# davdwan21/Silent-Speech

Hardware: AMD Instinct MI355X
Metric: clips/sec (30-frame, fwd+bwd) (higher is better)
Workload: dtype f32; 1 GPU; BASELINE config 2: landmark (K=40, D=84) + 64x64 uint8 ROI CNN + 2-layer BiGRU(192), T=30, C=5, train step = fwd + CE(ls .05) + bwd + grad all-reduce + clip(1.0) + Adam, dropout on; batch_per_gpu=256, global_batch=256, frames=30, parallelism=dp1, micro_batches_in_flight=1

## Files before the change

### silent_speech_amd/csrc/gemm.hip

```cpp
#include <stdlib.h>

#define SS_STAMP_ROW ((int)(blockIdx.x + gridDim.x * (blockIdx.y + gridDim.y * blockIdx.z)))
#include "ss_common.h"

STAMP_TABLE(ss_debug_stamps_gemm)

namespace {

constexpr int BM = 128, BN = 64, BK = 16;
constexpr int LDK = BK + 4;
constexpr int LDM_A = BM + 4;
constexpr int LDM_B = BN + 4;

struct RowMap {
  int G, S, off;
  __device__ __forceinline__ long operator()(int r) const {
    if (G == 0x7fffffff) return r + off;
    return (long)(r / G) * S + (r % G) + off;
  }
};

struct GemmParams {
  const float* A;
  const float* B;
  float* C;
  const float* bias;
  int M, N, K;
  int lda, ldb, ldc;
  RowMap ra, rb;
  float* asum;
  int ksplit;
  int nz;
  long sA, sB, sC, sBias, sAsum;
  int kcat;
  int flags;
};

struct TileId { int bx, by, bz, gx, gy; };

__device__ __forceinline__ void gemm_epilogue(const GemmParams& p, f32x4 (&acc)[4][2], int m0, int n0, int zs, int wm, int wn,
                                              int i, int g, float* stage ,
                                              const TileId& id) {
  if (p.flags & 8) {
    f32x4* w = reinterpret_cast<f32x4*>(p.C) + (((long)id.bz * id.gy + id.by) * id.gx + id.bx) * (8 * 256) + threadIdx.x;
#pragma unroll
    for (int mt = 0; mt < 4; ++mt)
#pragma unroll
      for (int nt = 0; nt < 2; ++nt) w[(mt * 2 + nt) * 256] = acc[mt][nt];
    return;
  }
  const bool accumulate = p.flags & 1, relu = p.flags & 2;
  const bool atomic = p.nz > 1 || (p.flags & 4);
  auto emit = [&](const f32x4& av, int mt, int nt) {
    int col = n0 + wn * 32 + nt * 16 + i;
    if (col >= p.N) return;
    float bv = (p.bias && zs == 0) ? p.bias[col] : 0.f;
#pragma unroll
    for (int r = 0; r < 4; ++r) {
      int row = m0 + wm * 64 + mt * 16 + 4 * g + r;
      if (row >= p.M) continue;
      float v = av[r] + bv;
      float* dst = p.C + (long)row * p.ldc + col;
      if (atomic) {
        atomicAdd(dst, v);
      } else {
        if (accumulate) v += *dst;
        if (relu) v = relu_f(v);
        *dst = v;
      }
    }
  };
  if (stage && !atomic && n0 + BN <= p.N && (p.ldc & 3) == 0 && (reinterpret_cast<uintptr_t>(p.C) & 15) == 0) {
    constexpr int LDS_C = BN + 4;
    __syncthreads();
#pragma unroll
    for (int mt = 0; mt < 4; ++mt)
#pragma unroll
      for (int nt = 0; nt < 2; ++nt) {
        const int col = wn * 32 + nt * 16 + i;
        const float bv = (p.bias && zs == 0) ? p.bias[n0 + col] : 0.f;
#pragma unroll
        for (int r = 0; r < 4; ++r) stage[(wm * 64 + mt * 16 + 4 * g + r) * LDS_C + col] = acc[mt][nt][r] + bv;
      }
    __syncthreads();
    const int c4 = (threadIdx.x & 15) * 4, r0 = threadIdx.x >> 4;
#pragma unroll
    for (int it = 0; it < BM / 16; ++it) {
      const int row = r0 + 16 * it;
      if (m0 + row < p.M) {
        f32x4 v = *reinterpret_cast<const f32x4*>(&stage[row * LDS_C + c4]);
        f32x4* dst = reinterpret_cast<f32x4*>(p.C + (long)(m0 + row) * p.ldc + n0 + c4);
        if (accumulate) v += *dst;
        if (relu) {
#pragma unroll
          for (int e = 0; e < 4; ++e) v[e] = relu_f(v[e]);
        }
        *dst = v;
      }
    }
    return;
  }
// ... 380 lines not shown
    }
  }
  if (rem) {
    __syncthreads();
    da.tail(dlds, rem);
    db.tail(dlds + D_A, rem);
    __syncthreads();
    compute(dlds, -1);
  }
  }
  static_assert(BM * (BN + 4) <= DSTAGES * D_STAGE, "the output tile is staged in the k-tile ring");
  gemm_epilogue(p, acc, m0, n0, zs, wm, wn, i, g, dlds, id);
}

template <bool A_KC, bool B_KC>
__global__ __launch_bounds__(256, 3) void gemm_dma_kernel(GemmParams p) {
  extern __shared__ __attribute__((aligned(16))) float dlds[];
  gemm_dma_body<A_KC, B_KC>(p, TileId{(int)blockIdx.x, (int)blockIdx.y, (int)blockIdx.z, (int)gridDim.x, (int)gridDim.y}, dlds);
}

constexpr int GEMM_GROUP_MAX = 4;
struct GemmGroup {
  GemmParams p[GEMM_GROUP_MAX];
  int first[GEMM_GROUP_MAX + 1];
  int gx[GEMM_GROUP_MAX], gy[GEMM_GROUP_MAX];
  int n;
};

template <bool A_KC, bool B_KC>
__global__ __launch_bounds__(256, 3) void gemm_dma_group_kernel(GemmGroup gg) {
  extern __shared__ __attribute__((aligned(16))) float dlds[];
  int j = 0;
#pragma unroll
  for (int q = 1; q < GEMM_GROUP_MAX; ++q)
    if (q < gg.n && (int)blockIdx.x >= gg.first[q]) j = q;
  const int local = blockIdx.x - gg.first[j], gx = gg.gx[j], gy = gg.gy[j];
  const int bx = local % gx, by = (local / gx) % gy, bz = local / (gx * gy);
  gemm_dma_body<A_KC, B_KC>(gg.p[j], TileId{bx, by, bz, gx, gy}, dlds);
}

struct ReduceItem { const f32x4* ws; int nz, gx, gy, M, N; float* C; int ldc; long sC; };
struct ReduceGroup {
  ReduceItem it[GEMM_GROUP_MAX];
  int first[GEMM_GROUP_MAX + 1];
  int n;
};
__device__ __forceinline__ void splitk_reduce_body(const ReduceItem& r, int block) {
  const int q = block & 7, tile = block >> 3;
  const int bx = tile % r.gx, by = (tile / r.gx) % r.gy, bi = tile / (r.gx * r.gy);
  const int tid = threadIdx.x, lane = tid & 63, wid = tid >> 6, wm = wid >> 1, wn = wid & 1, i = lane & 15, g = lane >> 4;
  const int mt = q >> 1, nt = q & 1;
  const f32x4* src = r.ws + ((((long)bi * r.nz) * r.gy + by) * r.gx + bx) * (8 * 256) + q * 256 + tid;
  const long zstride = (long)r.gy * r.gx * (8 * 256);
  f32x4 s0 = {0.f, 0.f, 0.f, 0.f};
  int z = 0;
  for (; z + 8 <= r.nz; z += 8) {
    f32x4 v[8];
#pragma unroll
    for (int u = 0; u < 8; ++u) v[u] = src[(z + u) * zstride];
    s0 += ((v[0] + v[1]) + (v[2] + v[3])) + ((v[4] + v[5]) + (v[6] + v[7]));
  }
  {
    f32x4 v[8];
#pragma unroll
    for (int u = 0; u < 8; ++u) v[u] = (z + u < r.nz) ? src[(z + u) * zstride] : f32x4{0.f, 0.f, 0.f, 0.f};
    s0 += ((v[0] + v[1]) + (v[2] + v[3])) + ((v[4] + v[5]) + (v[6] + v[7]));
  }
  const int col = bx * BN + wn * 32 + nt * 16 + i;
  if (col >= r.N) return;
#pragma unroll
  for (int rr = 0; rr < 4; ++rr) {
    const int row = by * BM + wm * 64 + mt * 16 + 4 * g + rr;
    if (row < r.M) r.C[bi * r.sC + (long)row * r.ldc + col] += s0[rr];
  }
}
__global__ __launch_bounds__(256) void splitk_reduce_kernel(ReduceItem r) { splitk_reduce_body(r, blockIdx.x); }
__global__ __launch_bounds__(256) void splitk_reduce_group_kernel(ReduceGroup rg) {
  int j = 0;
#pragma unroll
  for (int q = 1; q < GEMM_GROUP_MAX; ++q)
    if (q < rg.n && (int)blockIdx.x >= rg.first[q]) j = q;
  splitk_reduce_body(rg.it[j], blockIdx.x - rg.first[j]);
}

namespace wide {
constexpr int WT = 192, WNT = 512, WNWV = 8;
constexpr int W_U = WT / 4;
constexpr int W_PIECES = WT * BK / 4 / 64;
constexpr int W_STAGE = 2 * WT * BK;
constexpr int W_LPW = 2 * W_PIECES / WNWV;
constexpr int W_Q = 18;
constexpr int W_SLAB = WT * WT;
static_assert(2 * W_PIECES % WNWV == 0, "pieces deal evenly over the waves");

struct WideProblem {
  const float *A, *B;
  float* C;
  int M, N, K, lda, ldb, ldc;
  RowMap ra, rb;
  int ksplit, nz, gx, gy, batch;
  long sA, sB, sC;
  long ws_off;
};
struct WideGroup {
  WideProblem p[GEMM_GROUP_MAX];
  int first[GEMM_GROUP_MAX + 1];
  int rfirst[GEMM_GROUP_MAX + 1];
  float* ws;
  int n;
};

#define WIDE_K_LOOP                                                                                                      \
  {                                                                                                                      \
    _Pragma("unroll") for (int s_ = 0; s_ < DSTAGES - 1; ++s_) if (s_ < nfull) issue(s_);                                \
    for (int t0 = 0; t0 < nfull; t0 += DSTAGES) {                                                                        \
      _Pragma("unroll") for (int s_ = 0; s_ < DSTAGES; ++s_) {                                                           \
        const int t = t0 + s_;                                                                                           \
        if (t < nfull) {                                                                                                 \
          if (t + DSTAGES - 2 < nfull) ss_vmcnt_wait<(DSTAGES - 2) * W_LPW>(); else ss_vmcnt_wait<0>();                  \
          ss_raw_barrier();                                                                                              \
          if (t + DSTAGES - 1 < nfull) issue((s_ + DSTAGES - 1) % DSTAGES);                                              \
          read(dlds + s_ * W_STAGE);                                                                                     \
          mma();                                                                                                         \
        }                                                                                                                \
      }                                                                                                                  \
    }                                                                                                                    \
  }

struct WidePieces {
  const float* src[W_LPW];
  int q[W_LPW], r[W_LPW];
  int G[W_LPW], S[W_LPW], ld[W_LPW];
  bool lin[W_LPW];
  __device__ __forceinline__ void init(const WideProblem& P, const float* A, const float* B, int m0, int n0, int kbeg) {
    const int lane = threadIdx.x & 63, wave = threadIdx.x >> 6;
#pragma unroll
    for (int n = 0; n < W_LPW; ++n) {
      const int piece = wave + WNWV * n;
      const bool isb = piece >= W_PIECES;
      const int sl = (piece - (isb ? W_PIECES : 0)) * 64 + lane;
      const int k = sl / W_U, u = sl % W_U;
      int ru = u - 4 * ((k >> 2) & 1);
      ru += ru < 0 ? W_U : 0;
      const RowMap& rm = isb ? P.rb : P.ra;
      const int nrows = isb ? P.N : P.M, row0 = isb ? n0 : m0;
      ld[n] = isb ? P.ldb : P.lda;
      lin[n] = rm.G == 0x7fffffff;
      G[n] = rm.G; S[n] = rm.S;
      const int gk = kbeg + k;
      src[n] = (isb ? B : A) + min(row0 + 4 * ru, nrows - 4) + (long)rm.off * ld[n];
      q[n] = lin[n] ? 0 : gk / rm.G;
      r[n] = gk - q[n] * rm.G;
      if (lin[n]) src[n] += (long)gk * ld[n];
    }
  }
  __device__ __forceinline__ const float* cur(int n) const { return lin[n] ? src[n] : src[n] + ((long)q[n] * S[n] + r[n]) * ld[n]; }
  __device__ __forceinline__ void issue(unsigned stage_byte) const {
    const int wave = threadIdx.x >> 6;
#pragma unroll
    for (int n = 0; n < W_LPW; ++n) ss_dma16(cur(n), stage_byte + (wave + WNWV * n) * 1024);
  }
  __device__ __forceinline__ void advance() {
#pragma unroll
// ... 38 lines not shown
  dp.init(P, P.A + bi * P.sA, P.B + bi * P.sB, m0, n0, kbeg);
  int offA[3], offB[6];
#pragma unroll
  for (int mt = 0; mt < 3; ++mt) {
    const int m = wm * 48 + mt * 16 + i;
    offA[mt] = 4 * g * WT + 4 * (((m >> 2) + 4 * (g & 1)) % W_U) + (m & 3);
  }
#pragma unroll
  for (int nt = 0; nt < 6; ++nt) {
    const int nn = wn * 96 + nt * 16 + i;
    offB[nt] = WT * BK + 4 * g * WT + 4 * (((nn >> 2) + 4 * (g & 1)) % W_U) + (nn & 3);
  }
  f32x4 acc[3][6];
#pragma unroll
  for (int mt = 0; mt < 3; ++mt)
#pragma unroll
    for (int nt = 0; nt < 6; ++nt) acc[mt][nt] = f32x4{0.f, 0.f, 0.f, 0.f};

  auto issue = [&](int buf) {
    dp.issue((unsigned)(buf * W_STAGE * 4));
    dp.advance();
  };
  float a[3][4], b[6][4];
  auto read = [&](const float* st) {
#pragma unroll
    for (int kk = 0; kk < 4; ++kk) {
#pragma unroll
      for (int mt = 0; mt < 3; ++mt) a[mt][kk] = st[offA[mt] + kk * WT];
#pragma unroll
      for (int nt = 0; nt < 6; ++nt) b[nt][kk] = st[offB[nt] + kk * WT];
    }
  };
  auto mma = [&]() {
#pragma unroll
    for (int kk = 0; kk < 4; ++kk)
#pragma unroll
      for (int mt = 0; mt < 3; ++mt)
#pragma unroll
        for (int nt = 0; nt < 6; ++nt) acc[mt][nt] = mfma16(a[mt][kk], b[nt][kk], acc[mt][nt]);
  };
  WIDE_K_LOOP
  if (rem) {
    __syncthreads();
    dp.tail(dlds, rem);
    __syncthreads();
    read(dlds);
    mma();
  }
  f32x4* w = reinterpret_cast<f32x4*>(gg.ws + P.ws_off) + (long)local * (W_Q * WNT) + threadIdx.x;
#pragma unroll
  for (int mt = 0; mt < 3; ++mt)
#pragma unroll
    for (int nt = 0; nt < 6; ++nt) w[(mt * 6 + nt) * WNT] = acc[mt][nt];
}

__global__ __launch_bounds__(WNT) void gemm_wide_reduce_kernel(WideGroup gg) {
  int j = 0;
#pragma unroll
  for (int q = 1; q < GEMM_GROUP_MAX; ++q)
    if (q < gg.n && (int)blockIdx.x >= gg.rfirst[q]) j = q;
  const WideProblem& P = gg.p[j];
  const int blk = blockIdx.x - gg.rfirst[j];
  const int q = blk % W_Q, tile = blk / W_Q;
  const int bx = tile % P.gx, by = (tile / P.gx) % P.gy, bi = tile / (P.gx * P.gy);
  const int tid = threadIdx.x, lane = tid & 63, wid = tid >> 6, wm = wid >> 1, wn = wid & 1, i = lane & 15, g = lane >> 4;
  const int mt = q / 6, nt = q % 6;
  const long tiles = (long)P.gx * P.gy;
  const f32x4* src = reinterpret_cast<const f32x4*>(gg.ws + P.ws_off) + (((long)bi * P.nz * tiles + by * P.gx + bx) * W_Q + q) * WNT + tid;
  const long zstride = tiles * W_Q * WNT;
  f32x4 s0 = {0.f, 0.f, 0.f, 0.f};
  int z = 0;
  for (; z + 8 <= P.nz; z += 8) {
    f32x4 v[8];
#pragma unroll
    for (int u = 0; u < 8; ++u) v[u] = src[(z + u) * zstride];
    s0 += ((v[0] + v[1]) + (v[2] + v[3])) + ((v[4] + v[5]) + (v[6] + v[7]));
  }
  {
    f32x4 v[8];
#pragma unroll
    for (int u = 0; u < 8; ++u) v[u] = (z + u < P.nz) ? src[(z + u) * zstride] : f32x4{0.f, 0.f, 0.f, 0.f};
    s0 += ((v[0] + v[1]) + (v[2] + v[3])) + ((v[4] + v[5]) + (v[6] + v[7]));
  }
  const int col = bx * WT + wn * 96 + nt * 16 + i;
  if (col >= P.N) return;
#pragma unroll
  for (int rr = 0; rr < 4; ++rr) {
    const int row = by * WT + wm * 48 + mt * 16 + 4 * g + rr;
    if (row < P.M) P.C[bi * P.sC + (long)row * P.ldc + col] += s0[rr];
  }
}

struct WideKcParams {
  const float *A, *B, *bias;
  float* C;
  int M, N, K, lda, ldb, ldc, gx, gy;
  long sA, sB, sC, sBias;
};
struct WidePiecesKc {
  const float* src[W_LPW];
  __device__ __forceinline__ void init(const WideKcParams& P, const float* A, const float* B, int m0, int n0) {
    const int lane = threadIdx.x & 63, wave = threadIdx.x >> 6;
#pragma unroll
    for (int n = 0; n < W_LPW; ++n) {
      const int piece = wave + WNWV * n;
      const bool isb = piece >= W_PIECES;
      const int sl = (piece - (isb ? W_PIECES : 0)) * 64 + lane;
      const int rr = sl >> 2, ku = (sl & 3) ^ kc_swz(rr);
      const int nrows = isb ? P.N : P.M, row0 = isb ? n0 : m0;
      const int gr = min(row0 + rr, nrows - 1);
      src[n] = (isb ? B + (long)gr * P.ldb : A + (long)gr * P.lda) + 4 * ku;
    }
  }
  __device__ __forceinline__ void issue(unsigned stage_byte) const {
    const int wave = threadIdx.x >> 6;
#pragma unroll
    for (int n = 0; n < W_LPW; ++n) ss_dma16(src[n], stage_byte + (wave + WNWV * n) * 1024);
  }
  __device__ __forceinline__ void advance() {
#pragma unroll
    for (int n = 0; n < W_LPW; ++n) src[n] += BK;
  }
  __device__ __forceinline__ void tail(float* img, int kvalid) const {
    const int lane = threadIdx.x & 63, wave = threadIdx.x >> 6;
#pragma unroll
    for (int n = 0; n < W_LPW; ++n) {
      const int piece = wave + WNWV * n;
      const int sl = (piece % W_PIECES) * 64 + lane;
      const int ku = (sl & 3) ^ kc_swz(sl >> 2);
      f32x4 v = {0.f, 0.f, 0.f, 0.f};
#pragma unroll
      for (int e = 0; e < 4; ++e)
        if (4 * ku + e < kvalid) v[e] = src[n][e];
      *reinterpret_cast<f32x4*>(img + piece * 256 + 4 * lane) = v;
    }
  }
// ... 79 lines not shown
    }
  }
}
}

int splitk_slices(int K, int splits, int* per_out) {
  const int per = ceil_div(ceil_div(K, splits), BK * KSUB) * BK * KSUB;
  if (per_out) *per_out = per;
  return ceil_div(K, per);
}

}

extern "C" int ss_gemm_splitk_ws_floats(int M, int N, int K, int splits, int batch, long* floats) {
  SS_REQUIRE(M > 0 && N > 0 && K > 0 && splits >= 1 && batch >= 1 && floats, SS_ERR_ARG);
  *floats = (long)batch * splitk_slices(K, splits, nullptr) * ceil_div(M, BM) * ceil_div(N, BN) * BM * BN;
  return SS_OK;
}

extern "C" int ss_gemm_splitk_reduce(const float* ws, int M, int N, int K, int splits, int batch, float* C, int ldc,
                                     long stride_c, ss_stream_t stream) {
  SS_REQUIRE(ws && C && M > 0 && N > 0 && K > 0 && splits >= 1 && batch >= 1 && ldc >= N, SS_ERR_ARG);
  SS_REQUIRE((reinterpret_cast<uintptr_t>(ws) & 15) == 0, SS_ERR_ARG);
  const int nz = splitk_slices(K, splits, nullptr), gx = ceil_div(N, BN), gy = ceil_div(M, BM);
  const ReduceItem r{reinterpret_cast<const f32x4*>(ws), nz, gx, gy, M, N, C, ldc, stride_c};
  hipLaunchKernelGGL(splitk_reduce_kernel, dim3((unsigned)(batch * gx * gy * 8)), dim3(256), 0, static_cast<hipStream_t>(stream), r);
  return ss_launch_status();
}

struct GemmLaunch {
  GemmParams p;
  dim3 grid;
  bool dma_ok;
};
static int gemm_prepare(int a_kcontig, int b_kcontig, int M, int N, int K, const float* A, int lda, int a_group, int a_gstride,
                        int a_off, const float* B, int ldb, int b_group, int b_gstride, int b_off, float* C, int ldc,
                        const float* bias, float* a_colsum, int flags, int splits, int batch, long stride_a, long stride_b,
                        long stride_c, long stride_bias, long stride_colsum, GemmLaunch* out) {
  SS_REQUIRE(M > 0 && N > 0 && K > 0 && A && B && C && batch >= 1, SS_ERR_ARG);
  SS_REQUIRE(!a_colsum || !a_kcontig, SS_ERR_ARG);
  SS_REQUIRE(splits >= 1 && a_group > 0 && b_group > 0, SS_ERR_ARG);
  SS_REQUIRE((flags & 8) || (splits == 1 && !(flags & 4)) || ((flags & 1) && !(flags & 2)), SS_ERR_ARG);
  SS_REQUIRE(!(flags & 8) || (!(flags & 7) && !bias && (reinterpret_cast<uintptr_t>(C) & 15) == 0), SS_ERR_ARG);
  GemmParams& p = out->p;
  p.A = A; p.B = B; p.C = C; p.bias = bias; p.asum = a_colsum;
  p.M = M; p.N = N; p.K = K;
  p.lda = lda; p.ldb = ldb; p.ldc = ldc;
  p.ra = RowMap{a_group, a_gstride, a_off};
  p.rb = RowMap{b_group, b_gstride, b_off};
  p.nz = splitk_slices(K, splits, &p.ksplit);
  p.sA = stride_a; p.sB = stride_b; p.sC = stride_c; p.sBias = stride_bias; p.sAsum = stride_colsum;
  p.flags = flags & 15;
  p.kcat = 1;
  out->grid = dim3(ceil_div(N, BN), ceil_div(M, BM), p.nz * batch);
  SS_REQUIRE(out->grid.z <= 65535, SS_ERR_UNSUPPORTED);
  auto al16 = [](const void* q) { return (reinterpret_cast<uintptr_t>(q) & 15) == 0; };
  out->dma_ok = !a_colsum && al16(A) && al16(B) && (lda & 3) == 0 && (ldb & 3) == 0 && (stride_a & 3) == 0 &&
                (stride_b & 3) == 0 && (a_kcontig || (M >= 4 && (M & 3) == 0)) && (b_kcontig || (N >= 4 && (N & 3) == 0)) &&
                p.ksplit >= 4 * BK;
  return SS_OK;
}

extern "C" int ss_gemm_f32_batched(int a_kcontig, int b_kcontig, int M, int N, int K, const float* A, int lda,
                                   int a_group, int a_gstride, int a_off, const float* B, int ldb, int b_group,
                                   int b_gstride, int b_off, float* C, int ldc, const float* bias, float* a_colsum,
                                   int flags, int splits, int batch, long stride_a, long stride_b, long stride_c,
                                   long stride_bias, long stride_colsum, ss_stream_t stream) {
  GemmLaunch gl;
  const int st = gemm_prepare(a_kcontig, b_kcontig, M, N, K, A, lda, a_group, a_gstride, a_off, B, ldb, b_group, b_gstride, b_off,
                              C, ldc, bias, a_colsum, flags, splits, batch, stride_a, stride_b, stride_c, stride_bias,
                              stride_colsum, &gl);
  if (st != SS_OK) return st;
  GemmParams& p = gl.p;
  dim3 grid = gl.grid, block(256);
  const bool dma_ok = gl.dma_ok;
  hipStream_t s = static_cast<hipStream_t>(stream);
  if (flags & 16) {
    SS_REQUIRE(!(flags & 8) && !a_colsum, SS_ERR_ARG);
    if (!dma_ok) {
      for (int b = 0; b < batch; ++b) {
        const int st2 = ss_gemm_f32_batched(a_kcontig, b_kcontig, M, N, K, A + b * stride_a, lda, a_group, a_gstride, a_off,
                                            B + b * stride_b, ldb, b_group, b_gstride, b_off, C, ldc, b ? nullptr : bias, nullptr,
                                            (flags & 15) | (b ? 1 : 0), splits, 1, 0, 0, 0, 0, 0, stream);
        if (st2 != SS_OK) return st2;
      }
      return SS_OK;
    }
    p.kcat = batch;
    grid.z = p.nz;
  }
  if (dma_ok && a_kcontig && b_kcontig && !(flags & 31) && splits == 1 && p.ra.G == 0x7fffffff && p.ra.off == 0 &&
      p.rb.G == 0x7fffffff && p.rb.off == 0 && (K & 3) == 0) {
    const long tiles = (long)ceil_div(M, wide::WT) * ceil_div(N, wide::WT) * batch;
    const int cus = ss_device_cus();
    if (tiles <= cus && tiles * 10 >= (long)cus * 8 && N >= 96) {
      wide::WideKcParams w;
      w.A = A; w.B = B; w.bias = bias; w.C = C; w.M = M; w.N = N; w.K = K; w.lda = lda; w.ldb = ldb; w.ldc = ldc;
      w.gx = ceil_div(N, wide::WT); w.gy = ceil_div(M, wide::WT);
      w.sA = stride_a; w.sB = stride_b; w.sC = stride_c; w.sBias = stride_bias;
      constexpr size_t wide_lds = (size_t)DSTAGES * wide::W_STAGE * sizeof(float);
      static bool attr_set = false;
      if (!attr_set) {
        if (hipFuncSetAttribute(reinterpret_cast<const void*>(wide::gemm_wide_kc_kernel), hipFuncAttributeMaxDynamicSharedMemorySize,
                                (int)wide_lds) != hipSuccess)
          return SS_ERR_LAUNCH;
        attr_set = true;
      }
      hipLaunchKernelGGL(wide::gemm_wide_kc_kernel, dim3((unsigned)(w.gx * w.gy), (unsigned)batch), dim3(wide::WNT), wide_lds, s, w);
      return ss_launch_status();
    }
  }
  if (dma_ok) {
    constexpr size_t lds_bytes = (size_t)DSTAGES * D_STAGE * sizeof(float);
    if (a_kcontig && b_kcontig) hipLaunchKernelGGL((gemm_dma_kernel<true, true>), grid, block, lds_bytes, s, p);
    else if (a_kcontig && !b_kcontig) hipLaunchKernelGGL((gemm_dma_kernel<true, false>), grid, block, lds_bytes, s, p);
    else if (!a_kcontig && b_kcontig) hipLaunchKernelGGL((gemm_dma_kernel<false, true>), grid, block, lds_bytes, s, p);
    else hipLaunchKernelGGL((gemm_dma_kernel<false, false>), grid, block, lds_bytes, s, p);
    return ss_launch_status();
  }
  if (a_kcontig && b_kcontig) hipLaunchKernelGGL((gemm_f32_kernel<true, true>), grid, block, 0, s, p);
  else if (a_kcontig && !b_kcontig) hipLaunchKernelGGL((gemm_f32_kernel<true, false>), grid, block, 0, s, p);
  else if (!a_kcontig && b_kcontig) hipLaunchKernelGGL((gemm_f32_kernel<false, true>), grid, block, 0, s, p);
  else hipLaunchKernelGGL((gemm_f32_kernel<false, false>), grid, block, 0, s, p);
  return ss_launch_status();
}

static long group_ws_offset(const ss_gemm_problem* pr, int j) {
  long off = 0;
  for (int q = 0; q < j; ++q)
    off += (long)pr[q].batch * splitk_slices(pr[q].K, pr[q].splits, nullptr) * ceil_div(pr[q].M, BM) * ceil_div(pr[q].N, BN) * BM * BN;
  return off;
}

static bool wide_plan(const ss_gemm_problem* pr, int n, wide::WideGroup* out, long* floats) {
  using namespace wide;
  long work = 0;
  for (int j = 0; j < n; ++j) work += (long)ceil_div(pr[j].M, WT) * ceil_div(pr[j].N, WT) * pr[j].batch * pr[j].K;
  long kt = work / ss_device_cus() > 4 * BK ? work / ss_device_cus() : 4 * BK;
  auto slices = [&](int K, long kt_, int* ksplit) {
    int nz = (int)((K + kt_ / 2) / kt_);
    nz = nz < 1 ? 1 : nz;
    int ks = ceil_div(ceil_div(K, nz), BK) * BK;
    if (ks < 4 * BK) ks = 4 * BK;
    if (ksplit) *ksplit = ks;
    return ceil_div(K, ks);
  };
  for (int it = 0; it < 64; ++it) {
    long wgs = 0;
    for (int j = 0; j < n; ++j) wgs += (long)ceil_div(pr[j].M, WT) * ceil_div(pr[j].N, WT) * pr[j].batch * slices(pr[j].K, kt, nullptr);
    if (wgs <= ss_device_cus()) break;
    kt += kt / 32 + 1;
  }
  long off = 0;
  int first = 0, rfirst = 0;
  for (int j = 0; j < n; ++j) {
    const ss_gemm_problem& q = pr[j];
    WideProblem w;
    w.A = q.A; w.B = q.B; w.C = q.C;
    w.M = q.M; w.N = q.N; w.K = q.K; w.lda = q.lda; w.ldb = q.ldb; w.ldc = q.ldc;
    w.ra = RowMap{q.a_group, q.a_gstride, q.a_off};
    w.rb = RowMap{q.b_group, q.b_gstride, q.b_off};
    w.nz = slices(q.K, kt, &w.ksplit);
    w.gx = ceil_div(q.N, WT); w.gy = ceil_div(q.M, WT); w.batch = q.batch;
    w.sA = q.stride_a; w.sB = q.stride_b; w.sC = q.stride_c;
    w.ws_off = off;
    const int wgs = w.gx * w.gy * w.batch * w.nz;
    off += (long)wgs * W_SLAB;
    if (out) {
      out->p[j] = w;
      out->first[j] = first; out->rfirst[j] = rfirst;
    }
    first += wgs;
    rfirst += w.gx * w.gy * w.batch * W_Q;
  }
  if (out) {
    out->n = n;
    for (int j = n; j <= GEMM_GROUP_MAX; ++j) { out->first[j] = first; out->rfirst[j] = rfirst; }
    for (int j = n; j < GEMM_GROUP_MAX; ++j) out->p[j] = out->p[0];
  }
  if (floats) *floats = off;
  auto al16 = [](const void* q) { return (reinterpret_cast<uintptr_t>(q) & 15) == 0; };
  bool ok = true;
  for (int j = 0; j < n; ++j) {
    const ss_gemm_problem& q = pr[j];
    ok = ok && !q.a_kcontig && !q.b_kcontig && al16(q.A) && al16(q.B) && (q.lda & 3) == 0 && (q.ldb & 3) == 0 &&
         (q.stride_a & 3) == 0 && (q.stride_b & 3) == 0 && q.M >= 4 && (q.M & 3) == 0 && q.N >= 4 && (q.N & 3) == 0;
  }
  return ok;
}

extern "C" int ss_gemm_splitk_group_ws_floats(const ss_gemm_problem* problems, int n, long* floats) {
  SS_REQUIRE(problems && floats && n >= 1 && n <= GEMM_GROUP_MAX, SS_ERR_ARG);
  for (int j = 0; j < n; ++j)
    SS_REQUIRE(problems[j].M > 0 && problems[j].N > 0 && problems[j].K > 0 && problems[j].splits >= 1 && problems[j].batch >= 1,
               SS_ERR_ARG);
  long wide_floats = 0;
  wide_plan(problems, n, nullptr, &wide_floats);
  const long narrow = group_ws_offset(problems, n);
  *floats = wide_floats > narrow ? wide_floats : narrow;
  return SS_OK;
}

extern "C" int ss_gemm_f32_splitk_group(const ss_gemm_problem* problems, int n, float* ws, long ws_floats, int flags, ss_stream_t stream) {
  SS_REQUIRE(problems && ws && n >= 1 && n <= GEMM_GROUP_MAX, SS_ERR_ARG);
  {
    long need = 0;
    const int st = ss_gemm_splitk_group_ws_floats(problems, n, &need);
    if (st != SS_OK) return st;
    SS_REQUIRE(ws_floats >= need, SS_ERR_ARG);
  }
  SS_REQUIRE((reinterpret_cast<uintptr_t>(ws) & 15) == 0, SS_ERR_ARG);
  {
    wide::WideGroup wg;
    if ((flags & 1) && wide_plan(problems, n, &wg, nullptr)) {
      for (int j = 0; j < n; ++j) SS_REQUIRE(problems[j].C && problems[j].ldc >= problems[j].N, SS_ERR_ARG);
      wg.ws = ws;
      static bool attr_set = false;
      constexpr size_t wide_lds = (size_t)DSTAGES * wide::W_STAGE * sizeof(float);
      if (!attr_set) {
        if (hipFuncSetAttribute(reinterpret_cast<const void*>(wide::gemm_wide_group_kernel),
                                hipFuncAttributeMaxDynamicSharedMemorySize, (int)wide_lds) != hipSuccess)
          return SS_ERR_LAUNCH;
        attr_set = true;
      }
      hipStream_t s = static_cast<hipStream_t>(stream);
      hipLaunchKernelGGL(wide::gemm_wide_group_kernel, dim3((unsigned)wg.first[n]), dim3(wide::WNT), wide_lds, s, wg);
      if (ss_launch_status() != SS_OK) return SS_ERR_LAUNCH;
      hipLaunchKernelGGL(wide::gemm_wide_reduce_kernel, dim3((unsigned)wg.rfirst[n]), dim3(wide::WNT), 0, s, wg);
      return ss_launch_status();
    }
  }
  GemmGroup gg;
  ReduceGroup rg;
  gg.n = rg.n = n;
  gg.first[0] = rg.first[0] = 0;
  bool grouped = true;
  for (int j = 0; j < n; ++j) {
    const ss_gemm_problem& q = problems[j];
    GemmLaunch gl;
    float* wsj = ws + group_ws_offset(problems, j);
    const int st = gemm_prepare(q.a_kcontig, q.b_kcontig, q.M, q.N, q.K, q.A, q.lda, q.a_group, q.a_gstride, q.a_off, q.B, q.ldb,
                                q.b_group, q.b_gstride, q.b_off, wsj, q.N, nullptr, nullptr, 8, q.splits, q.batch, q.stride_a,
                                q.stride_b, 0, 0, 0, &gl);
    if (st != SS_OK) return st;
    SS_REQUIRE(q.C && q.ldc >= q.N, SS_ERR_ARG);
    grouped = grouped && gl.dma_ok && q.a_kcontig == problems[0].a_kcontig && q.b_kcontig == problems[0].b_kcontig;
    gg.p[j] = gl.p;
    gg.gx[j] = gl.grid.x; gg.gy[j] = gl.grid.y;
    gg.first[j + 1] = gg.first[j] + (int)(gl.grid.x * gl.grid.y * gl.grid.z);
    rg.it[j] = ReduceItem{reinterpret_cast<const f32x4*>(wsj), gl.p.nz, (int)gl.grid.x, (int)gl.grid.y, q.M, q.N, q.C, q.ldc, q.stride_c};
    rg.first[j + 1] = rg.first[j] + (int)(q.batch * gl.grid.x * gl.grid.y * 8);
  }
  for (int j = n; j < GEMM_GROUP_MAX; ++j) {
    gg.p[j] = gg.p[0]; gg.gx[j] = gg.gy[j] = 1; gg.first[j + 1] = gg.first[n];
    rg.it[j] = rg.it[0]; rg.first[j + 1] = rg.first[n];
  }
  hipStream_t s = static_cast<hipStream_t>(stream);
  if (!grouped) {
    for (int j = 0; j < n; ++j) {
      const ss_gemm_problem& q = problems[j];
      float* wsj = ws + group_ws_offset(problems, j);
      int st = ss_gemm_f32_batched(q.a_kcontig, q.b_kcontig, q.M, q.N, q.K, q.A, q.lda, q.a_group, q.a_gstride, q.a_off, q.B,
                                   q.ldb, q.b_group, q.b_gstride, q.b_off, wsj, q.N, nullptr, nullptr, 8, q.splits, q.batch,
                                   q.stride_a, q.stride_b, 0, 0, 0, stream);
      if (st != SS_OK) return st;
      st = ss_gemm_splitk_reduce(wsj, q.M, q.N, q.K, q.splits, q.batch, q.C, q.ldc, q.stride_c, stream);
      if (st != SS_OK) return st;
    }
    return SS_OK;
  }
  constexpr size_t lds_bytes = (size_t)DSTAGES * D_STAGE * sizeof(float);
  const dim3 ggrid((unsigned)gg.first[n]), block(256);
  const bool akc = problems[0].a_kcontig, bkc = problems[0].b_kcontig;
  if (akc && bkc) hipLaunchKernelGGL((gemm_dma_group_kernel<true, true>), ggrid, block, lds_bytes, s, gg);
  else if (akc && !bkc) hipLaunchKernelGGL((gemm_dma_group_kernel<true, false>), ggrid, block, lds_bytes, s, gg);
  else if (!akc && bkc) hipLaunchKernelGGL((gemm_dma_group_kernel<false, true>), ggrid, block, lds_bytes, s, gg);
  else hipLaunchKernelGGL((gemm_dma_group_kernel<false, false>), ggrid, block, lds_bytes, s, gg);
  if (ss_launch_status() != SS_OK) return SS_ERR_LAUNCH;
  hipLaunchKernelGGL(splitk_reduce_group_kernel, dim3((unsigned)rg.first[n]), dim3(256), 0, s, rg);
  return ss_launch_status();
}

extern "C" int ss_gemm_f32(int a_kcontig, int b_kcontig, int M, int N, int K, const float* A, int lda, int a_group,
                           int a_gstride, int a_off, const float* B, int ldb, int b_group, int b_gstride, int b_off,
                           float* C, int ldc, const float* bias, float* a_colsum, int flags, int splits,
                           ss_stream_t stream) {
  return ss_gemm_f32_batched(a_kcontig, b_kcontig, M, N, K, A, lda, a_group, a_gstride, a_off, B, ldb, b_group,
                             b_gstride, b_off, C, ldc, bias, a_colsum, flags, splits, 1, 0, 0, 0, 0, 0, stream);
}
```

### silent_speech_amd/engine.py

```python
from __future__ import annotations

import os

from dataclasses import dataclass
from typing import Dict, Optional

import torch

from . import _lib as L

INT_MAX = 2**31 - 1
_HH_TARGET = 512
USE_SIDE_STREAM = True


@dataclass
class Config:
    x_dim: int
    num_classes: int
    use_roi: bool
    roi_emb: int = 32
    hidden: int = 192
    gru_layers: int = 2
    roi_standardize: bool = True
    gru_dropout: float = 0.1
    head_dropout: float = 0.2
    head_mid: int = 128
    ln_eps: float = 1e-5
    cnn_channels: tuple = (8, 16, 24)
    precision: str = "f32"

    @property
    def in_dim(self) -> int:
        return self.x_dim + (self.roi_emb if self.use_roi else 0)


def gemm(a_kc, b_kc, M, N, K, A, lda, B, ldb, Cm, ldc, bias=None, accumulate=False, relu=False, splits=1,
         a_map=(INT_MAX, 0, 0), b_map=(INT_MAX, 0, 0), a_colsum=None, tag="gemm", batch=1, strides=(0, 0, 0, 0, 0),
         atomic=False, splitk_ws: Optional[torch.Tensor] = None, sum_batch=False):
    if splitk_ws is not None and splits > 1 and accumulate and not relu and bias is None:
        need = L.gemm_splitk_ws_floats(M, N, K, splits, batch)
        if splitk_ws.numel() < need:
            raise RuntimeError(f"split-K workspace too small: {splitk_ws.numel()} < {need}")
        L.call("ss_gemm_f32_batched", int(a_kc), int(b_kc), M, N, K, A, lda, a_map[0], a_map[1], a_map[2], B, ldb,
               b_map[0], b_map[1], b_map[2], splitk_ws.data_ptr(), N, None, a_colsum, 8, splits, batch,
               strides[0], strides[1], 0, 0, strides[4], L.stream(), tag=tag)
        L.call("ss_gemm_splitk_reduce", splitk_ws.data_ptr(), M, N, K, splits, batch, Cm, ldc, strides[2], L.stream(),
               tag=tag + "_reduce")
        return
    flags = (1 if accumulate else 0) | (2 if relu else 0) | (4 if atomic else 0) | (16 if sum_batch else 0)
    L.call("ss_gemm_f32_batched", int(a_kc), int(b_kc), M, N, K, A, lda, a_map[0], a_map[1], a_map[2], B, ldb,
           b_map[0], b_map[1], b_map[2], Cm, ldc, bias, a_colsum, flags, splits, batch, *strides, L.stream(), tag=tag)


_SPLITK_TARGET = 768
DW_WIDE_ALONE = 1
SKIP_PADDED_FRAMES = os.environ.get("SS_CNN_SKIP_PADDING", "1") != "0"

_DX_SPLIT_CAP = 2


def split_k(M, N, K, batch=1, target_wgs=_SPLITK_TARGET):
    tiles = -(-M // 128) * -(-N // 64) * batch
    return max(1, min(K // 128, target_wgs // tiles))


def dw_shapes(cfg, B, T, l):
    H, N = cfg.hidden, B * T
    K = cfg.in_dim if l == 0 else 2 * H
    out = [(3 * H, K, N, split_k(3 * H, K, N, 2))]
    if T > 1:
        Kh = B * (T - 1)
        out += [(2 * H, H, Kh, split_k(2 * H, H, Kh, 2, _HH_TARGET)), (H, H, Kh, split_k(H, H, Kh, 2, _HH_TARGET))]
    return out


def dw_problems(ws, G, cfg, l, lin, ld_in):
    B, T, H = ws.B, ws.T, cfg.hidden
    N, K = B * T, (cfg.in_dim if l == 0 else 2 * H)
    dg = ws.dG[l].data_ptr()
    wi, wir = f"gru.weight_ih_l{l}", f"gru.weight_ih_l{l}_reverse"
    wh, whr = f"gru.weight_hh_l{l}", f"gru.weight_hh_l{l}_reverse"
    ident = (INT_MAX, 0, 0)

    def prob(M, Nn, Kk, A, B_, Cm, ldc, splits, a_map, b_map, sa, sb, sc):
        return L.GemmProblem(0, 0, M, Nn, Kk, A, 4 * H, a_map[0], a_map[1], a_map[2], B_, ld_in if b_map is ident else 2 * H,
                             b_map[0], b_map[1], b_map[2], Cm, ldc, splits, 2, sa, sb, sc)

    shapes = dw_shapes(cfg, B, T, l)
    out = [prob(*shapes[0][:3], dg, lin, G[wi].data_ptr(), K, shapes[0][3], ident, ident, N * 4 * H, 0, _pstride(G, wi, wir))]
    if T > 1:
        am, bm = (T - 1, T, 1), (T - 1, T, 0)
        sa, sb, sc = N * 4 * H - 4 * H, H + 2 * H, _pstride(G, wh, whr)
        gw, hp = G[wh], ws.out[l].data_ptr()
        out.append(prob(*shapes[1][:3], dg, hp, gw.data_ptr(), H, shapes[1][3], am, bm, sa, sb, sc))
        out.append(prob(*shapes[2][:3], dg + 3 * H * 4, hp, _addr(gw, 2 * H * H), H, shapes[2][3], am, bm, sa, sb, sc))
    return out


def _pstride(P, a: str, b: str) -> int:
    return (P[b].data_ptr() - P[a].data_ptr()) // 4


def _addr(t: torch.Tensor, offset_elems: int = 0) -> int:
    return t.data_ptr() + offset_elems * t.element_size()


def zero_buffers(bufs) -> None:
    bufs = [b for b in bufs if b is not None and b.numel()]
# ... 22 lines not shown


def make_workspace(cfg: Config, B: int, T: int, roi_hw, device, train: bool, slot=0):
    if cfg.precision == "bf16":
        from .engine_bf16 import WorkspaceBf16

        return WorkspaceBf16(cfg, B, T, roi_hw, device, train, slot)
    return Workspace(cfg, B, T, roi_hw, device, train, slot)


class Workspace:

    bf16 = False

    def __init__(self, cfg: Config, B: int, T: int, roi_hw, device, train: bool, slot=0):
        self.cfg, self.B, self.T, self.roi_hw, self.train = cfg, B, T, roi_hw, train
        self.stash_gen, self.stash_live = 0, False
        N, H = B * T, cfg.hidden
        f32 = dict(device=device, dtype=torch.float32)
        u8 = dict(device=device, dtype=torch.uint8)
        self.lengths = torch.empty(B, device=device, dtype=torch.int32)
        nb = L.gru_sync_bytes(B, T, H)
        self.gru_sync = torch.zeros(nb // 4, device=device, dtype=torch.int32) if nb else None
        self.side = side_stream(device, slot) if train else None
        self.ev_fork = torch.cuda.Event() if train else None
        self.ev_join = torch.cuda.Event() if train else None
        self.ev_cnn_fwd = torch.cuda.Event() if train else None
        self.stagger = False
        self.Z = torch.empty(N, cfg.in_dim, **f32) if cfg.use_roi and roi_hw is not None else None
        self.cnn_generic = None
        if cfg.use_roi and roi_hw is not None:
            from . import cnn_generic

            if not cnn_generic.fused_supported(*roi_hw):
                self.cnn_generic = cnn_generic.GenericCnn(N, roi_hw[0], roi_hw[1], device, train)
        self.gi = [torch.empty(2, N, 3 * H, **f32) for _ in range(cfg.gru_layers)]
        self.out = [torch.empty(N, 2 * H, **f32) for _ in range(cfg.gru_layers)]
        self.attn = torch.empty(B, T, **f32)
        self.pooled = torch.empty(B, 2 * H, **f32)
        self.ln = torch.empty(B, 2 * H, **f32)
        self.mid = torch.empty(B, cfg.head_mid, **f32)
        self.logits = torch.empty(B, cfg.num_classes, **f32)
        self.out_drop = [torch.empty(N, 2 * H, **f32) for _ in range(cfg.gru_layers - 1)]
        self.mid_drop = torch.empty(B, cfg.head_mid, **f32)
        if train:
            self.save = [torch.empty(2, N, 4, H, **f32) for _ in range(cfg.gru_layers)]
            self.dG = [torch.empty(2, N, 4, H, **f32) for _ in range(cfg.gru_layers)]
            self.d_out = torch.empty(N, 2 * H, **f32)
            need = 0
            for l in range(cfg.gru_layers):
                probs = [L.GemmProblem(0, 0, m_, n_, k_, None, 0, 1, 0, 0, None, 0, 1, 0, 0, None, 0, sp_, 2, 0, 0, 0)
                         for (m_, n_, k_, sp_) in dw_shapes(cfg, B, T, l)]
                need = max(need, L.gemm_group_ws_floats(probs))
            self.splitk_ws = torch.empty(need, **f32)
            self.d_lower = [None] + [torch.empty(N, 2 * H, **f32) for _ in range(1, cfg.gru_layers)]
            self.ev_zero = torch.cuda.Event()
            self.xhat = torch.empty(B, 2 * H, **f32)
            self.rstd = torch.empty(B, **f32)
            self.d_logits = torch.empty(B, cfg.num_classes, **f32)
            self.d_mid = torch.empty(B, cfg.head_mid, **f32)
            self.tail_part = torch.empty(B, 3, 2 * H, **f32)
            self.d_ln = torch.empty(B, 2 * H, **f32)
            self.d_pooled = torch.empty(B, 2 * H, **f32)
            self.dZ = torch.empty(N, cfg.in_dim, **f32) if cfg.use_roi else None
            if cfg.use_roi and self.cnn_generic is None:
                Hh, Ww = roi_hw
                self.cnn_sizes = L.cnn_stash_sizes(Hh, Ww)
                n_a1, n_a2, n_i1, n_i2, n_m3, n_feat = self.cnn_sizes
                self.st_a1 = torch.empty(N, n_a1, **f32)
                self.st_i1 = torch.empty(N, n_i1, **u8)
                self.st_a2 = torch.empty(N, n_a2, **f32)
                self.st_i2 = torch.empty(N, n_i2, **u8)
                self.st_m3 = torch.empty(N, n_m3, **u8)
                self.st_feat = torch.empty(N, n_feat, **f32)
        self.frames = (torch.empty(1 + N, device=device, dtype=torch.int32)
                       if cfg.use_roi and roi_hw is not None and self.cnn_generic is None and SKIP_PADDED_FRAMES else None)
        self.frames_seen = (torch.full((1,), -1, dtype=torch.int32).pin_memory()
                            if self.frames is not None and train else None)
        self.walk_listed = self.frames is not None


def forward(P: Dict[str, torch.Tensor], cfg: Config, ws: Workspace, X: torch.Tensor, R: Optional[torch.Tensor], *,
            train: bool, stash: bool = False, seed: int = 0, ce=None, x_in_place: bool = False, z_ready: bool = False) -> torch.Tensor:
    if ws.bf16:
        from . import engine_bf16

        return engine_bf16.forward(P, cfg, ws, X, R, train=train, stash=stash, seed=seed, ce=ce, x_in_place=x_in_place)
    B, T, H, N = ws.B, ws.T, cfg.hidden, ws.B * ws.T
    s = L.stream()
    if stash and not ws.train:
        raise RuntimeError("stash=True needs a training workspace")
    if z_ready:
        if stash or train or not cfg.use_roi or X.shape[2] != cfg.in_dim:
            raise RuntimeError("z_ready: inference on rows of width in_dim = x_dim + roi_emb of a use_roi model")
        layer_in, ld_in = X.data_ptr(), cfg.in_dim
    elif cfg.use_roi:
        Hh, Ww = ws.roi_hw
        ws_Z = ws.Z
        if not x_in_place:
            L.call("ss_copy_rows_f32", X.data_ptr(), cfg.x_dim, ws_Z.data_ptr(), cfg.in_dim, N, cfg.x_dim, s)
        if ws.cnn_generic is not None:
            ws.cnn_generic.forward(P, R, cfg.roi_standardize, cfg.roi_emb, _addr(ws_Z, cfg.x_dim), cfg.in_dim, stash)
        else:
            cw = [P[k].data_ptr() for k in ("roi_cnn.net.0.weight", "roi_cnn.net.0.bias", "roi_cnn.net.3.weight",
                                            "roi_cnn.net.3.bias", "roi_cnn.net.6.weight", "roi_cnn.net.6.bias",
                                            "roi_cnn.fc.weight", "roi_cnn.fc.bias")]
            st = ([ws.st_a1.data_ptr(), ws.st_i1.data_ptr(), ws.st_a2.data_ptr(), ws.st_i2.data_ptr(),
# ... 57 lines not shown
    p_drop = cfg.head_dropout if train else 0.0
    top = ws.out[cfg.gru_layers - 1]
    L.call("ss_tail_bwd", top.data_ptr(), ws.lengths.data_ptr(), P["pool.score.weight"].data_ptr(),
           P["head.0.weight"].data_ptr(), P["head.1.weight"].data_ptr(), P["head.4.weight"].data_ptr(),
           ws.attn.data_ptr(), ws.xhat.data_ptr(), ws.rstd.data_ptr(), ws.mid.data_ptr(), d_logits.data_ptr(), B, T,
           2 * H, MID, C, p_drop, seed, 7 << 40, ws.d_mid.data_ptr(), ws.d_out.data_ptr(),
           G["head.0.weight"].data_ptr(), G["head.0.bias"].data_ptr(), G["pool.score.weight"].data_ptr(),
           G["pool.score.bias"].data_ptr(), ws.tail_part.data_ptr(), s)
    side = ws.side if USE_SIDE_STREAM else torch.cuda.current_stream()
    ws.ev_fork.record()

    def head_side_work():
        with torch.cuda.stream(side):
            side.wait_event(ws.ev_fork)
            zero_buffers(ws.d_lower[1:] + ([ws.dZ] if cfg.use_roi else []))
            ws.ev_zero.record()
            if ws.frames_seen is not None:
                ws.frames_seen.copy_(ws.frames[:1], non_blocking=True)
            for k_, name_ in enumerate(("head.0.weight", "head.0.bias", "pool.score.weight")):
                L.call("ss_colsum_f32", _addr(ws.tail_part, k_ * 2 * H), B, 2 * H, 3 * 2 * H, G[name_].data_ptr(), L.stream())
            gemm(0, 0, C, MID, B, d_logits.data_ptr(), C, ws.mid_drop.data_ptr(), MID, G["head.4.weight"].data_ptr(), MID,
                 accumulate=True, atomic=True, a_colsum=G["head.4.bias"].data_ptr())
            gemm(0, 0, MID, 2 * H, B, ws.d_mid.data_ptr(), MID, ws.ln.data_ptr(), 2 * H, G["head.1.weight"].data_ptr(),
                 2 * H, accumulate=True, atomic=True, a_colsum=G["head.1.bias"].data_ptr())

    use_drop = train and cfg.gru_dropout > 0.0
    zero_waited = False
    for l in range(cfg.gru_layers - 1, -1, -1):
        K = cfg.in_dim if l == 0 else 2 * H
        top_layer = l == cfg.gru_layers - 1
        g_in = ws.d_out if top_layer else ws.d_lower[l + 1]
        L.call("ss_gru_bwd", g_in.data_ptr(), ws.out[l].data_ptr(), ws.save[l].data_ptr(),
               P[f"gru.weight_hh_l{l}"].data_ptr(), P[f"gru.weight_hh_l{l}_reverse"].data_ptr(),
               ws.lengths.data_ptr(), B, T, H, ws.dG[l].data_ptr(),
               0.0 if (top_layer or not use_drop) else cfg.gru_dropout, seed, (l + 1) << 40,
               G[f"gru.bias_ih_l{l}"].data_ptr(), G[f"gru.bias_hh_l{l}"].data_ptr(),
               G[f"gru.bias_ih_l{l}_reverse"].data_ptr(), G[f"gru.bias_hh_l{l}_reverse"].data_ptr(), L.ptr(ws.gru_sync), s)
        if top_layer:
            head_side_work()
        if l == 0:
            if cfg.use_roi:
                lin, ld_in = ws.Z.data_ptr(), cfg.in_dim
            else:
                lin, ld_in = X.data_ptr(), cfg.x_dim
        else:
            use_drop = train and cfg.gru_dropout > 0.0
            lin, ld_in = (ws.out_drop[l - 1] if use_drop else ws.out[l - 1]).data_ptr(), 2 * H
        def side_work(l=l, K=K, lin=lin, ld_in=ld_in):
            side = ws.side if USE_SIDE_STREAM else torch.cuda.current_stream()
            ws.ev_fork.record()
            with torch.cuda.stream(side):
                side.wait_event(ws.ev_fork)
                L.call("ss_gemm_f32_splitk_group", *L.gemm_group(dw_problems(ws, G, cfg, l, lin, ld_in)), ws.splitk_ws.data_ptr(),
                       ws.splitk_ws.numel(), DW_WIDE_ALONE if l == 0 else 0, L.stream(), tag="gemm_gru_dW")
        if l == 0:
            side_work()
        need_dx = (l > 0) or cfg.use_roi or (d_X is not None)
        if need_dx:
            if l > 0:
                dst, ld_dst = ws.d_lower[l].data_ptr(), 2 * H
            elif cfg.use_roi:
                dst, ld_dst = ws.dZ.data_ptr(), cfg.in_dim
            else:
                dst, ld_dst = d_X.data_ptr(), cfg.x_dim
                zero_buffers([d_X])
            if not zero_waited:
                torch.cuda.current_stream().wait_event(ws.ev_zero)
                zero_waited = True
            wi, wir = f"gru.weight_ih_l{l}", f"gru.weight_ih_l{l}_reverse"
            c0 = cfg.x_dim if (l == 0 and cfg.use_roi and d_X is None) else 0
            tiles = -(-N // 128) * -(-(K - c0) // 64) * 2
            dx_splits = max(1, min(_DX_SPLIT_CAP, 768 // tiles, (3 * H) // 96))
            gemm(1, 0, N, K - c0, 3 * H, ws.dG[l].data_ptr(), 4 * H, _addr(P[wi], c0), K, dst + 4 * c0, ld_dst,
                 accumulate=True, atomic=True, tag="gemm_gru_dX", batch=2, splits=dx_splits,
                 strides=(N * 4 * H, _pstride(P, wi, wir), 0, 0, 0))
        if l > 0:
            side_work()
    side_joined = False
    if cfg.use_roi:
        Hh, Ww = ws.roi_hw
        if d_X is not None:
            L.call("ss_copy_rows_f32", ws.dZ.data_ptr(), cfg.in_dim, d_X.data_ptr(), cfg.x_dim, N, cfg.x_dim, s)
        if USE_SIDE_STREAM:
            ws.ev_join.record(ws.side)
            torch.cuda.current_stream().wait_event(ws.ev_join)
            side_joined = True
        names = ("roi_cnn.net.0.weight", "roi_cnn.net.0.bias", "roi_cnn.net.3.weight", "roi_cnn.net.3.bias",
                 "roi_cnn.net.6.weight", "roi_cnn.net.6.bias", "roi_cnn.fc.weight", "roi_cnn.fc.bias")
        if ws.cnn_generic is not None:
            ws.cnn_generic.backward(P, G, cfg.roi_emb, _addr(ws.dZ, cfg.x_dim), cfg.in_dim)
        else:
            L.call("ss_roi_cnn_bwd_frames", R.data_ptr(), N, Hh, Ww, int(cfg.roi_standardize), *[P[k].data_ptr() for k in names],
                   cfg.roi_emb, ws.st_a1.data_ptr(), ws.st_i1.data_ptr(), ws.st_a2.data_ptr(), ws.st_i2.data_ptr(),
                   ws.st_m3.data_ptr(), ws.st_feat.data_ptr(), ws.cnn_sizes.ptr, _addr(ws.dZ, cfg.x_dim), cfg.in_dim,
                   *[G[k].data_ptr() for k in names], L.ptr(ws.frames) if ws.walk_listed else None, s, tag="ss_roi_cnn_bwd")
    if USE_SIDE_STREAM and not side_joined:
        ws.ev_join.record(ws.side)
        torch.cuda.current_stream().wait_event(ws.ev_join)
```

Measured before the change: 134,100 clips/s.

## Fuse split-K reduction into GEMM via last-arriving-block counters

```diff
diff --git a/silent_speech_amd/csrc/gemm.hip b/silent_speech_amd/csrc/gemm.hip
--- a/silent_speech_amd/csrc/gemm.hip
+++ b/silent_speech_amd/csrc/gemm.hip
@@ -34,7 +34,46 @@
   long sA, sB, sC, sBias, sAsum;
   int kcat;
   int flags;
+  float* Cout;
+  unsigned* cnt;
 };
+
+__device__ __forceinline__ bool splitk_arrive_last(unsigned* cnt, int nz, float* flag) {
+  asm volatile("s_waitcnt vmcnt(0)" ::: "memory");
+  __syncthreads();
+  if (threadIdx.x == 0) {
+    __builtin_amdgcn_fence(__ATOMIC_RELEASE, "agent");
+    asm volatile("s_waitcnt vmcnt(0)" ::: "memory");
+    const unsigned seen = __hip_atomic_fetch_add(cnt, 1u, __ATOMIC_RELAXED, __HIP_MEMORY_SCOPE_AGENT);
+    const bool last = seen == (unsigned)(nz - 1);
+    if (last) {
+      __builtin_amdgcn_fence(__ATOMIC_ACQUIRE, "agent");
+      asm volatile("s_waitcnt vmcnt(0)" ::: "memory");
+      __hip_atomic_store(cnt, 0u, __ATOMIC_RELAXED, __HIP_MEMORY_SCOPE_AGENT);
+    }
+    *reinterpret_cast<volatile int*>(flag) = last ? 1 : 0;
+  }
+  __syncthreads();
+  return *reinterpret_cast<volatile int*>(flag) != 0;
+}
+
+__device__ __forceinline__ f32x4 splitk_slab_sum(const f32x4* src, long zstride, int nz) {
+  f32x4 s0 = {0.f, 0.f, 0.f, 0.f};
+  int z = 0;
+  for (; z + 8 <= nz; z += 8) {
+    f32x4 v[8];
+#pragma unroll
+    for (int u = 0; u < 8; ++u) v[u] = src[(z + u) * zstride];
+    s0 += ((v[0] + v[1]) + (v[2] + v[3])) + ((v[4] + v[5]) + (v[6] + v[7]));
+  }
+  {
+    f32x4 v[8];
+#pragma unroll
+    for (int u = 0; u < 8; ++u) v[u] = (z + u < nz) ? src[(z + u) * zstride] : f32x4{0.f, 0.f, 0.f, 0.f};
+    s0 += ((v[0] + v[1]) + (v[2] + v[3])) + ((v[4] + v[5]) + (v[6] + v[7]));
+  }
+  return s0;
+}
 
 struct TileId { int bx, by, bz, gx, gy; };
 
@@ -47,6 +86,23 @@
     for (int mt = 0; mt < 4; ++mt)
 #pragma unroll
       for (int nt = 0; nt < 2; ++nt) w[(mt * 2 + nt) * 256] = acc[mt][nt];
+    if (!(p.flags & 32)) return;
+    const int bi = id.bz / p.nz;
+    if (!splitk_arrive_last(p.cnt + ((long)bi * id.gy + id.by) * id.gx + id.bx, p.nz, stage)) return;
+    const f32x4* src = reinterpret_cast<const f32x4*>(p.C) + ((((long)bi * p.nz) * id.gy + id.by) * id.gx + id.bx) * (8 * 256) + threadIdx.x;
+    const long zstride = (long)id.gy * id.gx * (8 * 256);
+    float* Cb = p.Cout + bi * p.sC;
+#pragma unroll 1
+    for (int q = 0; q < 8; ++q) {
+      const f32x4 s0 = splitk_slab_sum(src + q * 256, zstride, p.nz);
+      const int col = n0 + wn * 32 + (q & 1) * 16 + i;
+      if (col >= p.N) continue;
+#pragma unroll
+      for (int r = 0; r < 4; ++r) {
+        const int row = m0 + wm * 64 + (q >> 1) * 16 + 4 * g + r;
+        if (row < p.M) Cb[(long)row * p.ldc + col] += s0[r];
+      }
+    }
     return;
   }
   const bool accumulate = p.flags & 1, relu = p.flags & 2;
@@ -533,20 +589,7 @@
   const int mt = q >> 1, nt = q & 1;
   const f32x4* src = r.ws + ((((long)bi * r.nz) * r.gy + by) * r.gx + bx) * (8 * 256) + q * 256 + tid;
   const long zstride = (long)r.gy * r.gx * (8 * 256);
-  f32x4 s0 = {0.f, 0.f, 0.f, 0.f};
-  int z = 0;
-  for (; z + 8 <= r.nz; z += 8) {
-    f32x4 v[8];
-#pragma unroll
-    for (int u = 0; u < 8; ++u) v[u] = src[(z + u) * zstride];
-    s0 += ((v[0] + v[1]) + (v[2] + v[3])) + ((v[4] + v[5]) + (v[6] + v[7]));
-  }
-  {
-    f32x4 v[8];
-#pragma unroll
-    for (int u = 0; u < 8; ++u) v[u] = (z + u < r.nz) ? src[(z + u) * zstride] : f32x4{0.f, 0.f, 0.f, 0.f};
-    s0 += ((v[0] + v[1]) + (v[2] + v[3])) + ((v[4] + v[5]) + (v[6] + v[7]));
-  }
+  const f32x4 s0 = splitk_slab_sum(src, zstride, r.nz);
   const int col = bx * BN + wn * 32 + nt * 16 + i;
   if (col >= r.N) return;
 #pragma unroll
@@ -582,14 +625,33 @@
   int ksplit, nz, gx, gy, batch;
   long sA, sB, sC;
   long ws_off;
+  int cnt_off;
 };
 struct WideGroup {
   WideProblem p[GEMM_GROUP_MAX];
   int first[GEMM_GROUP_MAX + 1];
   int rfirst[GEMM_GROUP_MAX + 1];
   float* ws;
+  unsigned* cnt;
   int n;
 };
+
+template <class Emit>
+__device__ __forceinline__ void wide_finish(const f32x4* src , long zstride, int nz, int m0, int n0,
+                                            int M, int N, Emit emit) {
+  const int tid = threadIdx.x, lane = tid & 63, wid = tid >> 6, wm = wid >> 1, wn = wid & 1, i = lane & 15, g = lane >> 4;
+#pragma unroll 1
+  for (int q = 0; q < W_Q; ++q) {
+    const f32x4 s0 = splitk_slab_sum(src + q * WNT + tid, zstride, nz);
+    const int col = n0 + wn * 96 + (q % 6) * 16 + i;
+    if (col >= N) continue;
+#pragma unroll
+    for (int rr = 0; rr < 4; ++rr) {
+      const int row = m0 + wm * 48 + (q / 6) * 16 + 4 * g + rr;
+      if (row < M) emit(row, col, s0[rr]);
+    }
+  }
+}
 
 #define WIDE_K_LOOP                                                                                                      \
   {                                                                                                                      \
@@ -734,6 +796,13 @@
   for (int mt = 0; mt < 3; ++mt)
 #pragma unroll
     for (int nt = 0; nt < 6; ++nt) w[(mt * 6 + nt) * WNT] = acc[mt][nt];
+  if (!gg.cnt) return;
+  const long tiles = (long)P.gx * P.gy;
+  if (!splitk_arrive_last(gg.cnt + P.cnt_off + bi * tiles + by * P.gx + bx, P.nz, dlds)) return;
+  float* Cb = P.C + bi * P.sC;
+  const int ldc = P.ldc;
+  wide_finish(reinterpret_cast<const f32x4*>(gg.ws + P.ws_off) + ((long)bi * P.nz * tiles + by * P.gx + bx) * (W_Q * WNT),
+              tiles * W_Q * WNT, P.nz, m0, n0, P.M, P.N, [&](int row, int col, float v) { Cb[(long)row * ldc + col] += v; });
 }
 
 __global__ __launch_bounds__(WNT) void gemm_wide_reduce_kernel(WideGroup gg) {
@@ -750,20 +819,7 @@
   const long tiles = (long)P.gx * P.gy;
   const f32x4* src = reinterpret_cast<const f32x4*>(gg.ws + P.ws_off) + (((long)bi * P.nz * tiles + by * P.gx + bx) * W_Q + q) * WNT + tid;
   const long zstride = tiles * W_Q * WNT;
-  f32x4 s0 = {0.f, 0.f, 0.f, 0.f};
-  int z = 0;
-  for (; z + 8 <= P.nz; z += 8) {
-    f32x4 v[8];
-#pragma unroll
-    for (int u = 0; u < 8; ++u) v[u] = src[(z + u) * zstride];
-    s0 += ((v[0] + v[1]) + (v[2] + v[3])) + ((v[4] + v[5]) + (v[6] + v[7]));
-  }
-  {
-    f32x4 v[8];
-#pragma unroll
-    for (int u = 0; u < 8; ++u) v[u] = (z + u < P.nz) ? src[(z + u) * zstride] : f32x4{0.f, 0.f, 0.f, 0.f};
-    s0 += ((v[0] + v[1]) + (v[2] + v[3])) + ((v[4] + v[5]) + (v[6] + v[7]));
-  }
+  const f32x4 s0 = splitk_slab_sum(src, zstride, P.nz);
   const int col = bx * WT + wn * 96 + nt * 16 + i;
   if (col >= P.N) return;
 #pragma unroll
@@ -949,6 +1005,7 @@
   p.sA = stride_a; p.sB = stride_b; p.sC = stride_c; p.sBias = stride_bias; p.sAsum = stride_colsum;
   p.flags = flags & 15;
   p.kcat = 1;
+  p.Cout = nullptr; p.cnt = nullptr;
   out->grid = dim3(ceil_div(N, BN), ceil_div(M, BM), p.nz * batch);
   SS_REQUIRE(out->grid.z <= 65535, SS_ERR_UNSUPPORTED);
   auto al16 = [](const void* q) { return (reinterpret_cast<uintptr_t>(q) & 15) == 0; };
@@ -1029,6 +1086,12 @@
   return off;
 }
 
+static long group_cnt_words(const ss_gemm_problem* pr, int n) {
+  long w = 0;
+  for (int j = 0; j < n; ++j) w += (long)pr[j].batch * ceil_div(pr[j].M, BM) * ceil_div(pr[j].N, BN);
+  return (w + 63) / 64 * 64;
+}
+
 static bool wide_plan(const ss_gemm_problem* pr, int n, wide::WideGroup* out, long* floats) {
   using namespace wide;
   long work = 0;
@@ -1049,7 +1112,7 @@
     kt += kt / 32 + 1;
   }
   long off = 0;
-  int first = 0, rfirst = 0;
+  int first = 0, rfirst = 0, cnt_off = 0;
   for (int j = 0; j < n; ++j) {
     const ss_gemm_problem& q = pr[j];
     WideProblem w;
@@ -1061,6 +1124,8 @@
     w.gx = ceil_div(q.N, WT); w.gy = ceil_div(q.M, WT); w.batch = q.batch;
     w.sA = q.stride_a; w.sB = q.stride_b; w.sC = q.stride_c;
     w.ws_off = off;
+    w.cnt_off = cnt_off;
+    cnt_off += w.gx * w.gy * w.batch;
     const int wgs = w.gx * w.gy * w.batch * w.nz;
     off += (long)wgs * W_SLAB;
     if (out) {
@@ -1094,7 +1159,7 @@
   long wide_floats = 0;
   wide_plan(problems, n, nullptr, &wide_floats);
   const long narrow = group_ws_offset(problems, n);
-  *floats = wide_floats > narrow ? wide_floats : narrow;
+  *floats = group_cnt_words(problems, n) + (wide_floats > narrow ? wide_floats : narrow);
   return SS_OK;
 }
 
@@ -1107,11 +1172,15 @@
     SS_REQUIRE(ws_floats >= need, SS_ERR_ARG);
   }
   SS_REQUIRE((reinterpret_cast<uintptr_t>(ws) & 15) == 0, SS_ERR_ARG);
+  unsigned* const cnt = reinterpret_cast<unsigned*>(ws);
+  const bool finish = flags & 2;
+  ws += group_cnt_words(problems, n);
   {
     wide::WideGroup wg;
     if ((flags & 1) && wide_plan(problems, n, &wg, nullptr)) {
       for (int j = 0; j < n; ++j) SS_REQUIRE(problems[j].C && problems[j].ldc >= problems[j].N, SS_ERR_ARG);
       wg.ws = ws;
+      wg.cnt = finish ? cnt : nullptr;
       static bool attr_set = false;
       constexpr size_t wide_lds = (size_t)DSTAGES * wide::W_STAGE * sizeof(float);
       if (!attr_set) {
@@ -1123,6 +1192,7 @@
       hipStream_t s = static_cast<hipStream_t>(stream);
       hipLaunchKernelGGL(wide::gemm_wide_group_kernel, dim3((unsigned)wg.first[n]), dim3(wide::WNT), wide_lds, s, wg);
       if (ss_launch_status() != SS_OK) return SS_ERR_LAUNCH;
+      if (finish) return SS_OK;
       hipLaunchKernelGGL(wide::gemm_wide_reduce_kernel, dim3((unsigned)wg.rfirst[n]), dim3(wide::WNT), 0, s, wg);
       return ss_launch_status();
     }
@@ -1143,6 +1213,11 @@
     SS_REQUIRE(q.C && q.ldc >= q.N, SS_ERR_ARG);
     grouped = grouped && gl.dma_ok && q.a_kcontig == problems[0].a_kcontig && q.b_kcontig == problems[0].b_kcontig;
     gg.p[j] = gl.p;
+    if (finish) {
+      gg.p[j].flags |= 32;
+      gg.p[j].Cout = q.C; gg.p[j].ldc = q.ldc; gg.p[j].sC = q.stride_c;
+      gg.p[j].cnt = cnt + (rg.first[j] >> 3);
+    }
     gg.gx[j] = gl.grid.x; gg.gy[j] = gl.grid.y;
     gg.first[j + 1] = gg.first[j] + (int)(gl.grid.x * gl.grid.y * gl.grid.z);
     rg.it[j] = ReduceItem{reinterpret_cast<const f32x4*>(wsj), gl.p.nz, (int)gl.grid.x, (int)gl.grid.y, q.M, q.N, q.C, q.ldc, q.stride_c};
@@ -1174,6 +1249,7 @@
   else if (!akc && bkc) hipLaunchKernelGGL((gemm_dma_group_kernel<false, true>), ggrid, block, lds_bytes, s, gg);
   else hipLaunchKernelGGL((gemm_dma_group_kernel<false, false>), ggrid, block, lds_bytes, s, gg);
   if (ss_launch_status() != SS_OK) return SS_ERR_LAUNCH;
+  if (finish) return SS_OK;
   hipLaunchKernelGGL(splitk_reduce_group_kernel, dim3((unsigned)rg.first[n]), dim3(256), 0, s, rg);
   return ss_launch_status();
 }
diff --git a/silent_speech_amd/engine.py b/silent_speech_amd/engine.py
--- a/silent_speech_amd/engine.py
+++ b/silent_speech_amd/engine.py
@@ -55,6 +55,7 @@
 
 _SPLITK_TARGET = 768
 DW_WIDE_ALONE = 1
+DW_FINISH = 2
 SKIP_PADDED_FRAMES = os.environ.get("SS_CNN_SKIP_PADDING", "1") != "0"
 
 _DX_SPLIT_CAP = 2
@@ -183,7 +184,7 @@
                 probs = [L.GemmProblem(0, 0, m_, n_, k_, None, 0, 1, 0, 0, None, 0, 1, 0, 0, None, 0, sp_, 2, 0, 0, 0)
                          for (m_, n_, k_, sp_) in dw_shapes(cfg, B, T, l)]
                 need = max(need, L.gemm_group_ws_floats(probs))
-            self.splitk_ws = torch.empty(need, **f32)
+            self.splitk_ws = torch.zeros(need, **f32)
             self.d_lower = [None] + [torch.empty(N, 2 * H, **f32) for _ in range(1, cfg.gru_layers)]
             self.ev_zero = torch.cuda.Event()
             self.xhat = torch.empty(B, 2 * H, **f32)
@@ -347,7 +348,7 @@
             with torch.cuda.stream(side):
                 side.wait_event(ws.ev_fork)
                 L.call("ss_gemm_f32_splitk_group", *L.gemm_group(dw_problems(ws, G, cfg, l, lin, ld_in)), ws.splitk_ws.data_ptr(),
-                       ws.splitk_ws.numel(), DW_WIDE_ALONE if l == 0 else 0, L.stream(), tag="gemm_gru_dW")
+                       ws.splitk_ws.numel(), DW_WIDE_ALONE if l == 0 else DW_FINISH, L.stream(), tag="gemm_gru_dW")
         if l == 0:
             side_work()
         need_dx = (l > 0) or cfg.use_roi or (d_X is not None)
```

After: 128,500 clips/s. -4.2%, worse.
